# 20k/geodesic_raytracing

Hardware: AMD Instinct MI355X
Metric: Mrays/sec at 3840x2160 Kerr (whole frame: prepass + init + adaptive Verlet + render-data + anisotropic render) (higher is better)
Workload: dtype f32; 1 GPU; kerr_boyer (Boyer-Lindquist rs=1 a=0.45) 3840x2160, camera (0,0,-4,0) fov 90, adaptive_sampling off, prepass on, tol 1e-06, background 4096x2048 RGBA8 10 mips, anisotropy 8; mode=fused, prepass_lookahead=True, prepass_lookahead_depth=1, frames_in_flight=3, prepass=look-ahead on side streams, priming_frames=0, build_key=c6224cf99bf5a7bd-v80s8, counters_tag=kerr_a045_4k, program=substituted (parameters baked in, metric_manager.hpp:153-166), parallelism=single GPU

## Files before the change

### __graft_entry__.py

```python
import os
import subprocess
import sys

ROOT = os.path.dirname(os.path.abspath(__file__))
if ROOT not in sys.path:
    sys.path.insert(0, ROOT)

CONFIG_METRICS = ["minkowski", "schwarzschild", "kerr_boyer", "alcubierre"]
SCRIPT_METRICS = ["minkowski", "schwarzschild", "schwarzschild_adaptive", "kerr_boyer", "double_unequal_kerr", "alcubierre"]


_PRECOMPILE = "import sys; sys.path.insert(0, sys.argv[1]); import geodesic_raytracing_amd as gra; gra.Program.precompile(sys.argv[2])"


def _precompile(job):
    env, argument_string = job
    r = subprocess.run([sys.executable, "-c", _PRECOMPILE, ROOT, argument_string], env=dict(os.environ, **env), capture_output=True, text=True)
    if r.returncode != 0:
        raise RuntimeError(f"precompile of {argument_string[:200]}... failed ({r.returncode}):\n{r.stdout[-2000:]}{r.stderr[-4000:]}")
    return True


def _host_cpus():
    if os.environ.get("MAX_JOBS", "").isdigit() and int(os.environ["MAX_JOBS"]) > 0:
        return int(os.environ["MAX_JOBS"])
    n = len(os.sched_getaffinity(0)) if hasattr(os, "sched_getaffinity") else (os.cpu_count() or 2)
    try:
        with open("/sys/fs/cgroup/cpu.max") as f:
            quota, period = f.read().split()[:2]
        if quota != "max":
            n = min(n, max(1, int(quota) // int(period)))
    except (OSError, ValueError):
        pass
    return n


def build():
    subprocess.check_call(["make", "-C", os.path.join(ROOT, "geodesic_raytracing_amd", "csrc"), "-j8"])
    import geodesic_raytracing_amd as gra
    subprocess.check_call(["make", "-C", os.path.join(ROOT, "examples")])

    cache = os.path.join(ROOT, "geodesic_raytracing_amd", "_cache")
    kernel_dir = os.path.join(ROOT, "geodesic_raytracing_amd", "csrc", "kernels")
    newest_source = max(os.path.getmtime(os.path.join(kernel_dir, f)) for f in os.listdir(kernel_dir))
    if os.path.isdir(cache):
        for f in os.listdir(cache):
            path = os.path.join(cache, f)
            if os.path.getmtime(path) < newest_source:
                os.remove(path)
    jobs = []

    class _Collect:
        @staticmethod
        def precompile(argument_string, **env):
            job = (dict(env), argument_string)
            if job not in jobs:
                jobs.append(job)
    compile_later = _Collect()
    for name in CONFIG_METRICS:
        m = gra.Metric(name)
        compile_later.precompile(m.argument_string())
    compile_later.precompile(gra.Metric("kerr_boyer").argument_string(), GR_TRACE_PAIR_BUILD="1")
    scripts = os.path.join(ROOT, "geodesic_raytracing_amd", "scripts")
    script_metrics = [gra.Metric(name, scripts) for name in SCRIPT_METRICS]
    for m in script_metrics:
        compile_later.precompile(m.argument_string())
        cfg = m.cfg_values(a=0.45) if m.name == "kerr_boyer" else m.cfg_values()
        compile_later.precompile(m.argument_string(features=m.features(adaptive_sampling=0), static=True, cfg_values=cfg))
        if m.name == "kerr_boyer":
            compile_later.precompile(m.argument_string(features=m.features(adaptive_sampling=1, adaptive_sampling_threshold=32.0), static=True, cfg_values=cfg))
        if m.name == "kerr_boyer":
            compile_later.precompile(m.argument_string(features=m.features(adaptive_sampling=0), static=True, cfg_values=m.cfg_values(a=0.9)))
        if m.name == "kerr_boyer":
            for spin in (0.45, 0.9):
                compile_later.precompile(m.argument_string(features=m.features(adaptive_sampling=0), static=True, cfg_values=m.cfg_values(a=spin)) + " -DGR_PARKING")
    import glob as _glob
    for js in sorted(_glob.glob(os.path.join(scripts, "*.js"))):
        m = gra.Metric(os.path.basename(js)[:-3], scripts)
        compile_later.precompile(m.argument_string())
        compile_later.precompile(m.argument_string(features=m.features(adaptive_sampling=1, adaptive_sampling_threshold=32.0), static=True, cfg_values=m.cfg_values()))
    for m in script_metrics:
        if m.name == "alcubierre":
            compile_later.precompile(m.argument_string(features=m.features(adaptive_sampling=0, redshift=1), static=True, cfg_values=m.cfg_values()))

    import glob
    import json
    import numpy as np
    seen = set()
    for f in sorted(glob.glob(os.path.join(ROOT, "tests", "golden", "refscripts", "*.npz"))):
        meta = json.loads(str(np.load(f, allow_pickle=False)["meta"]))
        for text in (meta["argument_string"], meta["argument_string_substituted"]):
            if text not in seen:
                seen.add(text)
                compile_later.precompile(text)
    for f in sorted(glob.glob(os.path.join(ROOT, "tests", "golden", "*.npz")) + glob.glob(os.path.join(ROOT, "tests", "golden", "paths", "*.npz")) + glob.glob(os.path.join(ROOT, "tests", "golden", "paths", "soak", "*.npz"))
                    + glob.glob(os.path.join(ROOT, "tests", "golden", "polar", "*.npz")) + glob.glob(os.path.join(ROOT, "tests", "golden", "soak", "*.npz"))):
        meta = json.loads(str(np.load(f, allow_pickle=False)["meta"]))
        key = (meta["metric"], bool(meta.get("scripts")))
        metric = gra.Metric(meta["metric"], scripts if key[1] else None)
        if key not in seen:
            seen.add(key)
            compile_later.precompile(metric.argument_string())
        if "width" in meta and meta["width"] > 1:
            substituted = metric.argument_string(features=gra.default_features(**meta["features"]), static=True, cfg_values=meta["cfg"])
            if substituted not in seen:
                seen.add(substituted)
                compile_later.precompile(substituted)
                if "near_extreme" in f:
                    compile_later.precompile(substituted + " -cl-fp32-correctly-rounded-divide-sqrt")
                    compile_later.precompile(substituted + " -DGR_REFINED_RECIPROCALS")
    import importlib.util
    spec = importlib.util.spec_from_file_location("fuzz_parity", os.path.join(ROOT, "tests", "fuzz_parity.py"))
    fuzz = importlib.util.module_from_spec(spec)
    spec.loader.exec_module(fuzz)
    fuzz_oracles = []
    for case in fuzz.draw_cases(11, 7):
        metric, cfg, fkw = case[2], case[3], case[7]
        for text in (metric.argument_string(), metric.argument_string(features=gra.default_features(**fkw), static=True, cfg_values=cfg)):
            if text not in seen:
                seen.add(text)
                compile_later.precompile(text)
        fuzz_oracles.append(metric.argument_string())
    spec = importlib.util.spec_from_file_location("uniform_wave_paths", os.path.join(ROOT, "tests", "test_gpu_uniform_wave_paths.py"))
    uniform = importlib.util.module_from_spec(spec)
    spec.loader.exec_module(uniform)
    for name, cfg, features, _position, _ordered, variant in uniform.CASES.values():
        text = uniform.substituted(name, cfg, **features)[3] + (variant[0] if variant else "")
        compile_later.precompile(text)
        compile_later.precompile(text + uniform.WITHOUT)
    tests_dir = os.path.join(ROOT, "tests")
    sys.path.insert(0, tests_dir)
    try:
        spec = importlib.util.spec_from_file_location("render_data_model", os.path.join(tests_dir, "render_data_model.py"))
        render_data_model = importlib.util.module_from_spec(spec)
        spec.loader.exec_module(render_data_model)
    finally:
        sys.path.remove(tests_dir)
    render_data_oracles = [render_data_model.ProgramOf(name).argument_string for name in render_data_model.PROGRAMS]
    for text in render_data_oracles:
        compile_later.precompile(text)
    from concurrent.futures import ThreadPoolExecutor
    workers = max(1, min(len(jobs), _host_cpus() - 1))
    with ThreadPoolExecutor(workers) as pool:
        done = list(pool.map(_precompile, jobs))
    assert all(done) and len(done) == len(jobs)

    from oracle import build_restate, build_ref
    for name in CONFIG_METRICS:
        build_restate.build(gra.Metric(name).argument_string())
    for m in script_metrics:
        build_restate.build(m.argument_string())
    for text in fuzz_oracles + render_data_oracles:
        build_restate.build(text)
    if build_ref.reference_available():
        for name in CONFIG_METRICS:
            build_ref.build_metric(name)
        for m in script_metrics:
            build_ref.build(m.name + "_script", m.argument_string())


def smoke():
    import ctypes
    import numpy as np
    import torch
    import geodesic_raytracing_amd as gra
    from oracle import build_restate
    from oracle.refpipe import OraclePipeline, pack_features

    assert torch.cuda.is_available(), "smoke() needs a GPU: the ray kernels have no CPU fallback"
    W, H = 96, 54
    metric = gra.Metric("kerr_boyer")
    cfg = metric.cfg_values(a=0.45)
    feats = metric.features(adaptive_sampling=0)
    program = gra.Program(metric.argument_string(), 0)
    state = gra.RenderState(W, H, 0)
    bg_np, levels = gra.pack_background(gra.synthetic_background(256, 128))
    device = torch.device("cuda", 0)
    bg = torch.from_numpy(bg_np).to(device)
    out = torch.zeros((H, W, 4), dtype=torch.float32, device=device)
    opts = gra.frame_options(mode=gra.MODE_FUSED, use_prepass=0)
    state.render(program, metric, gra.default_camera(), out.data_ptr(), (bg.data_ptr(), 256, 128, levels), feats, cfg, opts,
                 torch.cuda.current_stream().cuda_stream)
    torch.cuda.synchronize()
    gpu = out.cpu().numpy()

    pipe = OraclePipeline(build_restate.build(metric.argument_string()))
    ref = pipe.frame(W, H, cfg, pack_features(adaptive_sampling=0, max_acceleration_change=metric.info.max_acceleration_change),
                     use_prepass=False, background=(bg_np, levels), nthreads=os.cpu_count() or 1)
    diff = gpu[..., :3] - ref["pixels"][..., :3]
    bad = np.abs(diff).max(axis=2) > 1e-3
    rmse = float(np.sqrt((diff[~bad] ** 2).mean()))
    print(f"smoke: kerr {W}x{H} fused HIP frame vs CPU oracle: rmse {rmse:.2e}, masked {bad.mean() * 100:.2f}% of pixels")
    assert np.isfinite(gpu).all()
    assert bad.mean() <= 0.02, "more than 2% of pixels differ from the oracle by > 1e-3"
    assert rmse < 1e-4, "pixel RMSE vs oracle above 1e-4"


if __name__ == "__main__":
    build()
    print("build ok")
```

### geodesic_raytracing_amd/csrc/kernels/integrator.hip

```cpp

#ifdef ADAPTIVE_PRECISION
#define GR_W_MAX ((float)((W_V1 > W_V2 ? W_V1 : W_V2) > (W_V3 > W_V4 ? W_V3 : W_V4) ? (W_V1 > W_V2 ? W_V1 : W_V2) : (W_V3 > W_V4 ? W_V3 : W_V4)))

__device__ __forceinline__ float acceleration_to_precision(float4 acc, float max_acceleration, float& next_ds) {
    float4 wa = f4(acc.x * (float)(W_V1), acc.y * (float)(W_V2), acc.z * (float)(W_V3), acc.w * (float)(W_V4));
    float current = __builtin_sqrtf(dot4(wa, wa)) * 0.01f;
    current /= GR_W_MAX;
    const float scale = 65536.f;
    float err = max_acceleration;
    float diff = current * scale;
    float floor_diff = err * scale / 1e10f;
    if (diff < floor_diff) diff = floor_diff;
    next_ds = __builtin_sqrtf(err * scale) * __builtin_amdgcn_rsqf(diff);
    return diff;
}
#endif

enum { DS_NONE = 0, DS_SKIP = 1, DS_RETURN = 2 };

#ifdef GR_NO_UNIFORM_WAVE_PATHS
#define GR_UNIFORM_WAVE_PATHS 0
#else
#define GR_UNIFORM_WAVE_PATHS 1
#endif
#if GR_UNIFORM_WAVE_PATHS && defined(GR_RADIUS_EXITS_ORDERED) && !defined(GR_POLAR_R_SQUARED) && !(defined(GR_DISTANCE_SQUARED_OF_GENERIC) && defined(ADAPTIVE_PRECISION))
#define GR_OUTER_BOUNDARY_NEEDS_A_RAY_OUTSIDE 1
#else
#define GR_OUTER_BOUNDARY_NEEDS_A_RAY_OUTSIDE 0
#endif

struct ray_state {
    float4 position, velocity, acceleration;
    float next_ds;
    float running_dlambda_dnew;
    float f_in_x;
    int steps;
    unsigned int tries;
};

enum { RAY_LOST = 0, RAY_TERMINATED = 1 };

__device__ __forceinline__ void integrate_begin(ray_state& s, dfg_t dfg) {
    s.f_in_x = __builtin_fabsf(s.velocity.x);
    s.next_ds = 0.00001f;
#ifdef ADAPTIVE_PRECISION
    (void)acceleration_to_precision(s.acceleration, GET_FEATURE(max_acceleration_change, dfg), s.next_ds);
#endif
    s.running_dlambda_dnew = 1;
    s.steps = 0;
    s.tries = 0;
}

__device__ __forceinline__ float min_f32(float a, float b) { float r; asm("v_min_f32 %0, %1, %2" : "=v"(r) : "v"(a), "v"(b)); return r; }
__device__ __forceinline__ float max_f32(float a, float b) { float r; asm("v_max_f32 %0, %1, %2" : "=v"(r) : "v"(a), "v"(b)); return r; }

__device__ __forceinline__ void overwrite(float4& dst, float4 src) {
    asm volatile("v_mov_b32 %0, %4\n\tv_mov_b32 %1, %5\n\tv_mov_b32 %2, %6\n\tv_mov_b32 %3, %7"
                 : "+v"(dst.x), "+v"(dst.y), "+v"(dst.z), "+v"(dst.w) : "v"(src.x), "v"(src.y), "v"(src.z), "v"(src.w));
}

__device__ __forceinline__ float min_f32_uniform(float uniform, float x) { float r; asm("v_min_f32 %0, %1, %2" : "=v"(r) : "s"(uniform), "v"(x)); return r; }
__device__ __forceinline__ float max_f32_uniform(float uniform, float x) { float r; asm("v_max_f32 %0, %1, %2" : "=v"(r) : "s"(uniform), "v"(x)); return r; }

#ifdef ADAPTIVE_PRECISION
struct step_controller {
    float floor_q, root, singular_q, min_step;
    float root99, floor_step, ambient;
    __device__ __forceinline__ step_controller(float max_acceleration, float min_step_in, float ambient_in) {
        const float scale = 65536.f;
        const float floor_diff = max_acceleration * scale / 1e10f;
        floor_q = floor_diff * floor_diff;
        root = __builtin_sqrtf(max_acceleration * scale);
        root99 = 0.99f * root;
        const float singular = max_acceleration * 10000 * scale;
        singular_q = singular * singular;
        min_step = min_step_in;
        ambient = ambient_in;
        floor_step = __builtin_fminf(min_step_in, ambient_in);
    }
    __device__ __forceinline__ float raw_error_q(float4 acc) const {
        const float k = 0.01f * 65536.f / GR_W_MAX;
        const float wx = acc.x * (float)(W_V1), wy = acc.y * (float)(W_V2), wz = acc.z * (float)(W_V3), ww = acc.w * (float)(W_V4);
        const float d2 = __builtin_fmaf(wx, wx, __builtin_fmaf(wy, wy, __builtin_fmaf(wz, wz, ww * ww)));
        return d2 * (k * k);
    }
    __device__ __forceinline__ float error_q(float4 acc) const { return max_f32_uniform(floor_q, raw_error_q(acc)); }
    __device__ __forceinline__ float suggestion(float q) const { return root * __builtin_amdgcn_rsqf(__builtin_sqrtf(q)); }
    static constexpr bool error_sees_every_component = (float)(W_V1) != 0 && (float)(W_V2) != 0 && (float)(W_V3) != 0 && (float)(W_V4) != 0;
};
#endif

template <bool LIBM> struct trig_flavour { static constexpr bool value = LIBM; };

template <bool RESUMABLE, bool PARKABLE = false>
__device__ __forceinline__ int integrate_pingpong(ray_state& s, cfg_t cfg, dfg_t dfg, unsigned int* attempts, int keep_lanes, bool& paused,
                                                  bool resumed = false, unsigned int park_trips = 0) {
    float4 p0 = s.position, v0 = s.velocity, a0 = s.acceleration;
    float4 p1 = p0, v1 = v0, a1 = a0;
    const bool carried = RESUMABLE || (PARKABLE && resumed);
    if (PARKABLE && !resumed) { s.steps = 0; s.tries = 0; }
    const float f_in_x = carried ? s.f_in_x : __builtin_fabsf(v0.x);
    if (PARKABLE) s.f_in_x = f_in_x;
    const float subambient_precision = 0.5f;
    const float ambient_precision = 0.2f;
    float next_ds = 0.00001f;
#ifdef ADAPTIVE_PRECISION
    const step_controller controller(GET_FEATURE(max_acceleration_change, dfg), GET_FEATURE(min_step, dfg), ambient_precision);
    if (carried) next_ds = s.next_ds;
    else {
        float4 a = a0;
#ifdef IS_CONSTANT_THETA
        a.z = 0;
#endif
        next_ds = controller.suggestion(controller.error_q(a));
    }
    next_ds = min_f32_uniform(ambient_precision, next_ds);
#endif
    const float new_max = GET_FEATURE(max_precision_radius, dfg);
    const float new_min = 3;
    const float universe = GET_FEATURE(universe_size, dfg);
    const bool reparam = GET_FEATURE(reparameterisation, dfg) != 0;
    float running = carried ? s.running_dlambda_dnew : 1.f;
    const int loop_limit = 4096 * 4;
    const unsigned int budget_before = (unsigned int)(loop_limit - (carried ? s.steps : 0));
    unsigned int budget = budget_before;
    unsigned int rejections = 0;
    paused = false;

    auto stop_lost = [&](float4 pos, float4 vel, float4 acc, float run) {
        bool lost = false;
#ifdef HAS_CYLINDRICAL_SINGULARITY
        lost |= pos.y < CYLINDRICAL_TERMINATOR;
#endif
#ifndef UNCONDITIONALLY_NONSINGULAR
        bool runaway = __builtin_fabsf(vel.x / run) > 1000 + f_in_x;
        if (__builtin_expect(__builtin_amdgcn_ballot_w64(runaway) != 0, 0)) {
            asm volatile("; second condition of the runaway test");
            runaway = runaway && __builtin_fabsf(acc.x / run) > 100;
        }
        lost |= runaway;
#endif
        (void)pos; (void)vel; (void)acc; (void)run;
        return lost;
    };
#ifdef GR_POLAR_R_SQUARED
    const float universe2 = universe * universe;
    auto stop_terminated = [&](float4 position, float4 polar) {
        (void)polar;
        const float r2 = gm::polar_radius_squared(position, cfg);
        bool t = r2 >= universe2;
#ifdef SINGULAR
        t |= r2 < (float)(SINGULAR_TERMINATOR) * (float)(SINGULAR_TERMINATOR);
#endif
        return t;
    };
#else
    auto stop_terminated = [&](float4 position, float4 polar) {
        (void)position;
        bool t = __builtin_fabsf(polar.y) >= universe;
#ifdef SINGULAR
        t |= __builtin_fabsf(polar.y) < SINGULAR_TERMINATOR;
#endif
        return t;
    };
#endif
    const float far_offset = ambient_precision - 0.1f * new_max;
#if GR_UNIFORM_WAVE_PATHS
    auto outer_boundary_candidates = [&](float4 pos, float4 polar) {
#ifdef GR_POLAR_R_SQUARED
        (void)polar;
        return __builtin_amdgcn_ballot_w64(gm::polar_radius_squared(pos, cfg) >= universe2);
#else
        (void)pos;
        return __builtin_amdgcn_ballot_w64(__builtin_fabsf(polar.y) >= universe);
#endif
    };
    auto loop_top_candidates = [&](float4 pos, float4 vel, float4 polar, float run) {
        unsigned long long lanes = 0;
#ifdef HAS_CYLINDRICAL_SINGULARITY
        lanes |= __builtin_amdgcn_ballot_w64(pos.y < CYLINDRICAL_TERMINATOR);
#endif
#ifndef UNCONDITIONALLY_NONSINGULAR
        lanes |= __builtin_amdgcn_ballot_w64(__builtin_fabsf(vel.x / run) > 1000 + f_in_x);
#endif
#ifdef SINGULAR
#ifdef GR_POLAR_R_SQUARED
        lanes |= __builtin_amdgcn_ballot_w64(gm::polar_radius_squared(pos, cfg) < (float)(SINGULAR_TERMINATOR) * (float)(SINGULAR_TERMINATOR));
#else
        lanes |= __builtin_amdgcn_ballot_w64(__builtin_fabsf(polar.y) < SINGULAR_TERMINATOR);
#endif
#endif
#if !GR_OUTER_BOUNDARY_NEEDS_A_RAY_OUTSIDE
        lanes |= outer_boundary_candidates(pos, polar);
#endif
        (void)pos; (void)vel; (void)polar; (void)run;
        return lanes;
    };
#endif
    bool pause_wave = false;
    auto attempt = [&](auto libm, float4 position, float4 velocity, float4 acceleration, float4& po, float4& vo, float4& ao, float& ds_used,
                       float& running_before) -> bool {
        if (__builtin_expect(__builtin_usub_overflow(budget, 1u, &budget), 0)) return true;
#ifdef IS_CONSTANT_THETA
        position.z = GR_PIf / 2; velocity.z = 0; acceleration.z = 0;
#endif
        float4 polar = gm::generic_to_spherical(position, cfg);
#ifdef IS_CONSTANT_THETA
        polar.z = GR_PIf / 2;
#endif
#if defined(GR_DISTANCE_SQUARED_OF_GENERIC) && defined(ADAPTIVE_PRECISION)
        const float ar2 = gm::distance_squared_from(position, cfg);
        const bool inside = ar2 < new_max * new_max;
#else
        const float ar = __builtin_fabsf(gm::distance_to_object_from(position, polar, cfg));
        const bool inside = ar < new_max;
#endif
        const unsigned long long inside_lanes = __builtin_amdgcn_ballot_w64(inside);
        const bool wave_inside = inside_lanes != 0;
        (void)wave_inside;
#ifdef ADAPTIVE_PRECISION
        const float near_ds = next_ds;
#else
        const float near_ds = min_f32_uniform(ambient_precision, mixf(ambient_precision, subambient_precision, (clampf(ar, new_min, new_max) - new_min) / (new_max - new_min)));
#endif
#if GR_UNIFORM_WAVE_PATHS
        const bool wave_all_inside = inside_lanes == __builtin_amdgcn_ballot_w64(true);
        unsigned long long leaving = loop_top_candidates(position, velocity, polar, running);
        float ds = near_ds;
        if (!wave_all_inside) {
            asm volatile("; a ray outside the precision radius: the far step, the outer boundary");
#if defined(GR_DISTANCE_SQUARED_OF_GENERIC) && defined(ADAPTIVE_PRECISION)
            const float far_ds = __builtin_fmaf(0.1f, __builtin_sqrtf(ar2), far_offset);
#else
            const float far_ds = __builtin_fmaf(0.1f, ar, far_offset);
#endif
            ds = inside ? near_ds : far_ds;
#if GR_OUTER_BOUNDARY_NEEDS_A_RAY_OUTSIDE
            leaving |= outer_boundary_candidates(position, polar);
#endif
        }
        ds_used = ds;
        running_before = running;
        if (__builtin_expect(leaving != 0, 0)) {
            asm volatile("; a ray at a loop-top exit");
            if (stop_lost(position, velocity, acceleration, running) | stop_terminated(position, polar)) return true;
        }
#else
#if defined(GR_DISTANCE_SQUARED_OF_GENERIC) && defined(ADAPTIVE_PRECISION)
        float far_ds = near_ds;
        if (inside_lanes != __builtin_amdgcn_ballot_w64(true)) {
            asm volatile("; a ray outside the precision radius: the far step");
            far_ds = __builtin_fmaf(0.1f, __builtin_sqrtf(ar2), far_offset);
        }
#else
        const float far_ds = __builtin_fmaf(0.1f, ar, far_offset);
#endif
        const float ds = inside ? near_ds : far_ds;
        ds_used = ds;
        running_before = running;
        if (stop_lost(position, velocity, acceleration, running) | stop_terminated(position, polar)) return true;
#endif
        GR_PROBE_EXTRA_INSTRUCTIONS(ds)
        const float half_ds = 0.5f * ds, half_ds2 = half_ds * ds;
        const float4 next_position = position + velocity * ds + acceleration * half_ds2;
        const float4 predicted = velocity + acceleration * ds;
        float4 next_acceleration = GR_PROBE_ACCELERATION(gm::geodesic_acceleration_with<decltype(libm)::value>(next_position, predicted, cfg), acceleration, predicted, next_position);
        float4 next_velocity = velocity + (acceleration + next_acceleration) * half_ds;
        if (reparam) {
            const float md = __builtin_fmaxf(__builtin_fmaxf(__builtin_fabsf(next_velocity.x), __builtin_fabsf(next_velocity.y)),
                                             __builtin_fmaxf(__builtin_fabsf(next_velocity.z), __builtin_fabsf(next_velocity.w)));
            const float K = 1 / md;
            next_velocity = next_velocity * K;
            next_acceleration = next_acceleration * K * K;
            running *= K;
        }

        po = next_position;
        vo = next_velocity;
        ao = next_acceleration;
        bool dead = false;
#ifdef ADAPTIVE_PRECISION
        float q, nds1;
        unsigned long long rare_lanes;
        if (wave_inside) {
            q = controller.raw_error_q(next_acceleration);
            nds1 = __builtin_amdgcn_fmed3f(controller.root99 * __builtin_amdgcn_rsqf(__builtin_sqrtf(q)), (0.99f * 0.3f) * near_ds, (0.99f * 2.f) * near_ds);
            const float clamped = __builtin_amdgcn_fmed3f(nds1, controller.floor_step, controller.ambient);
            const float threshold = near_ds * (1 / 1.95f);
            rare_lanes = __builtin_amdgcn_ballot_w64(!(__builtin_fmaf(q, 0.f, clamped) >= threshold));
#ifdef SINGULARITY_DETECTION
            rare_lanes |= __builtin_amdgcn_ballot_w64(clamped == controller.floor_step);
#endif
            if (!step_controller::error_sees_every_component) {
                const float poison = (next_velocity.x + next_velocity.y) + (next_velocity.z + next_velocity.w);
                rare_lanes |= __builtin_amdgcn_ballot_w64(!(__builtin_fabsf(poison) <= 3.402823466e+38f));
            }
#if GR_UNIFORM_WAVE_PATHS
            next_ds = clamped;
            if (!wave_all_inside) {
                asm volatile("; a ray outside the precision radius keeps its carried step");
                next_ds = inside ? clamped : near_ds;
            }
#else
            next_ds = inside ? clamped : near_ds;
#endif
        } else {
            const float poison = (next_velocity.x + next_velocity.y) + (next_velocity.z + next_velocity.w);
            q = poison * 0.f;
            nds1 = 0;
            rare_lanes = __builtin_amdgcn_ballot_w64(!(q == q));
        }
        if (__builtin_expect(rare_lanes != 0, 0)) {
            asm volatile("; rejected step, singularity, degenerate state");
            const float nds = max_f32_uniform(controller.min_step, nds1);
#ifdef SINGULARITY_DETECTION
            dead = inside & (q > controller.singular_q) & (nds == controller.min_step);
#endif
            bool reject = inside & (nds < ds * (1 / 1.95f));
            bool degenerate = !(q == q);
            if (!step_controller::error_sees_every_component) {
                const float poison = (next_velocity.x + next_velocity.y) + (next_velocity.z + next_velocity.w);
                degenerate |= !(__builtin_fabsf(poison) <= 3.402823466e+38f);
            }
            dead |= !reject & degenerate;
#ifndef GR_ACCEL_WITHOUT_TRIG
            if (!decltype(libm)::value) {
                dead |= degenerate;
                reject &= !degenerate;
            }
#endif
            if (reject) {
                overwrite(po, position);
                overwrite(vo, velocity);
                overwrite(ao, acceleration);
                asm volatile("v_add_u32 %0, 1, %0\n\tv_add_u32 %1, 1, %1" : "+v"(rejections), "+v"(budget));
            }
        }
#else
        {
            const float poison = (next_velocity.x + next_velocity.y) + (next_velocity.z + next_velocity.w);
            dead = !(__builtin_fabsf(poison) <= 3.402823466e+38f);
        }
#endif
        if (__builtin_expect(dead, 0)) return true;
        if (RESUMABLE) {
            if (__builtin_popcountll(__builtin_amdgcn_ballot_w64(true)) < keep_lanes) { pause_wave = true; return true; }
        }
        return false;
    };

    float exit_ds = 0, exit_running = 1;
    {
        const trig_flavour<false> polynomial;
#if GR_PRIORITY_TRIPS > 0
        unsigned trips = 0, next_level = GR_PRIORITY_TRIPS;
#ifndef GR_PARK_PRIORITY
#define GR_PARK_PRIORITY 0
#endif
        if (PARKABLE && resumed) { __builtin_amdgcn_s_setprio(GR_PARK_PRIORITY); next_level = 0xffffffffu; }
#endif
        unsigned int visit_trips = 0;
        const int park_below = PARKABLE ? __builtin_amdgcn_readfirstlane(keep_lanes) : 0;
        const unsigned int park_after = PARKABLE ? __builtin_amdgcn_readfirstlane(park_trips) : 0u;
        for (;;) {
            float4 p1, v1, a1;
            float ds_used, running_before;
#if GR_PRIORITY_TRIPS > 0
            if (__builtin_expect(++trips == next_level, 0)) {
                if (next_level == GR_PRIORITY_TRIPS) __builtin_amdgcn_s_setprio(1);
                else if (next_level == 2 * GR_PRIORITY_TRIPS) __builtin_amdgcn_s_setprio(2);
                else __builtin_amdgcn_s_setprio(3);
                next_level = next_level < 4 * GR_PRIORITY_TRIPS ? 2 * next_level : 0xffffffffu;
            }
#endif
            if (attempt(polynomial, p0, v0, a0, p1, v1, a1, ds_used, running_before)) {
                if (RESUMABLE && pause_wave) { overwrite(p0, p1); overwrite(v0, v1); overwrite(a0, a1); }
                asm volatile("v_mov_b32 %0, %2\n\tv_mov_b32 %1, %3" : "+v"(exit_ds), "+v"(exit_running) : "v"(ds_used), "v"(running_before));
                break;
            }
            if (attempt(polynomial, p1, v1, a1, p0, v0, a0, ds_used, running_before)) {
                if (!(RESUMABLE && pause_wave)) { overwrite(p0, p1); overwrite(v0, v1); overwrite(a0, a1); }
                asm volatile("v_mov_b32 %0, %2\n\tv_mov_b32 %1, %3" : "+v"(exit_ds), "+v"(exit_running) : "v"(ds_used), "v"(running_before));
                break;
            }
            if (PARKABLE) {
                visit_trips = __builtin_amdgcn_readfirstlane(visit_trips) + 1u;
                if (__builtin_expect(visit_trips >= park_after && __builtin_popcountll(__builtin_amdgcn_ballot_w64(true)) < park_below, 0)) {
                    pause_wave = true;
                    break;
                }
            }
        }
    }
#if GR_PRIORITY_TRIPS > 0
    __builtin_amdgcn_s_setprio(0);
#endif
    float4 position = p0, velocity = v0, acceleration = a0;
#ifdef IS_CONSTANT_THETA
    position.z = GR_PIf / 2; velocity.z = 0; acceleration.z = 0;
#endif
    bool capped, lost_at_top, terminated_at_top;
    auto classify = [&]() {
        capped = budget == 0xffffffffu;
        float4 polar = gm::generic_to_spherical(position, cfg);
#ifdef IS_CONSTANT_THETA
        polar.z = GR_PIf / 2;
#endif
        lost_at_top = stop_lost(position, velocity, acceleration, running);
        terminated_at_top = stop_terminated(position, polar);
    };
    classify();
#if !defined(GR_FAST_TRIG) && !defined(GR_LIBM_TRIG) && !defined(GR_PROBE_NO_SLOW_TRIG)
    if (__builtin_expect(!capped && !pause_wave && !(lost_at_top | terminated_at_top), 0)) {
        const float ds_used = exit_ds;
        float4 polar = gm::generic_to_spherical(position, cfg);
        if (__builtin_fabsf(gm::distance_to_object_from(position, polar, cfg)) < new_max) next_ds = ds_used;
        running = exit_running;
        budget++;
        const trig_flavour<true> precise;
        for (;;) {
            float4 np, nv, na;
            float unused_ds, unused_running;
            const bool leave = attempt(precise, position, velocity, acceleration, np, nv, na, unused_ds, unused_running);
            if (leave && !pause_wave) break;
            position = np; velocity = nv; acceleration = na;
            if (leave) break;
        }
        classify();
    }
#endif
    paused = (RESUMABLE || PARKABLE) && pause_wave;
    const bool left_at_top = !capped && !paused && (lost_at_top | terminated_at_top);
    int result = RAY_LOST;
    if (!paused) {
        const bool finite = degenerate_accumulate(position, degenerate_accumulate(velocity, degenerate_accumulate(acceleration, 0.f))) == 0.f;
        if (!capped && !lost_at_top && terminated_at_top && finite) result = RAY_TERMINATED;
    }
    const unsigned int taken = capped ? budget_before : budget_before - budget - (left_at_top ? 1u : 0u);
    if (RESUMABLE || PARKABLE) { s.next_ds = next_ds; s.steps += (int)taken; s.tries += taken + rejections; }
    s.position = position;
    s.velocity = velocity;
    s.acceleration = acceleration;
    s.running_dlambda_dnew = running;
    if (attempts) *attempts = (RESUMABLE || PARKABLE) ? s.tries : taken + rejections;
    return result;
}

__device__ __forceinline__ int integrate_ray(ray_state& s, cfg_t cfg, dfg_t dfg, unsigned int* attempts) {
    bool paused;
    return integrate_pingpong<false>(s, cfg, dfg, attempts, 0, paused);
}


#ifdef GR_TWO_RAYS_PER_LANE
using gm::pairf;
using gm::pair4;
using gm::splat;
__device__ __forceinline__ pair4 operator+(pair4 a, pair4 b) { return {a.x + b.x, a.y + b.y, a.z + b.z, a.w + b.w}; }
__device__ __forceinline__ pair4 operator*(pair4 a, pairf s) { return {a.x * s, a.y * s, a.z * s, a.w * s}; }
template <int H> __device__ __forceinline__ float4 half_of(pair4 v) {
    return H == 0 ? f4(v.x.x, v.y.x, v.z.x, v.w.x) : f4(v.x.y, v.y.y, v.z.y, v.w.y);
}
__device__ __forceinline__ pair4 pair_of(float4 a, float4 b) {
    pair4 r;
    r.x.x = a.x; r.x.y = b.x; r.y.x = a.y; r.y.y = b.y; r.z.x = a.z; r.z.y = b.z; r.w.x = a.w; r.w.y = b.w;
    return r;
}

#ifdef ADAPTIVE_PRECISION
__device__ __forceinline__ pairf acceleration_to_precision(pair4 acc, float max_acceleration, pairf& next_ds) {
    pair4 wa = {acc.x * (float)(W_V1), acc.y * (float)(W_V2), acc.z * (float)(W_V3), acc.w * (float)(W_V4)};
    pairf d2 = wa.x * wa.x + wa.y * wa.y + wa.z * wa.z + wa.w * wa.w;
    pairf current;
    current.x = __builtin_sqrtf(d2.x); current.y = __builtin_sqrtf(d2.y);
    current = current * 0.01f;
    current = current / GR_W_MAX;
    const float scale = 65536.f;
    float err = max_acceleration;
    pairf diff = current * scale;
    float floor_diff = err * scale / 1e10f;
    if (diff.x < floor_diff) diff.x = floor_diff;
    if (diff.y < floor_diff) diff.y = floor_diff;
    const float root = __builtin_sqrtf(err * scale);
    next_ds.x = root * __builtin_amdgcn_rsqf(diff.x);
    next_ds.y = root * __builtin_amdgcn_rsqf(diff.y);
    return diff;
}
#endif

__device__ __forceinline__ void integrate_pair(pair4& position_io, pair4& velocity_io, pair4 acceleration, pairf& running_out,
                                               bool active0, bool active1, cfg_t cfg, dfg_t dfg, int& result0, int& result1,
                                               unsigned int& tries0, unsigned int& tries1) {
    pair4 position = position_io, velocity = velocity_io;
    pairf f_in_x;
    f_in_x.x = __builtin_fabsf(velocity.x.x); f_in_x.y = __builtin_fabsf(velocity.x.y);
#ifdef IS_CONSTANT_THETA
    position.z = splat(GR_PIf / 2); velocity.z = splat(0.f); acceleration.z = splat(0.f);
#endif
    pairf next_ds = splat(0.00001f);
#ifdef ADAPTIVE_PRECISION
    const float max_accel = GET_FEATURE(max_acceleration_change, dfg);
    const float min_step = GET_FEATURE(min_step, dfg);
    (void)acceleration_to_precision(acceleration, max_accel, next_ds);
#endif
    const float subambient_precision = 0.5f;
    const float ambient_precision = 0.2f;
    const float new_max = GET_FEATURE(max_precision_radius, dfg);
    const float new_min = 3;
    const float universe = GET_FEATURE(universe_size, dfg);
    const bool reparam = GET_FEATURE(reparameterisation, dfg) != 0;
    pairf running = splat(1.f);
    const int loop_limit = 4096 * 4;
    unsigned int t0 = 0, t1 = 0;
    int i0 = 0, i1 = 0;
    bool alive0 = active0, alive1 = active1;

    auto stop_lost = [&](float pos_y, float vel_x_over_run, float acc_x_over_run, float fin, int steps) {
        bool lost = steps >= loop_limit;
#ifdef HAS_CYLINDRICAL_SINGULARITY
        lost |= pos_y < CYLINDRICAL_TERMINATOR;
#endif
#ifndef UNCONDITIONALLY_NONSINGULAR
        lost |= __builtin_fabsf(vel_x_over_run) > 1000 + fin && __builtin_fabsf(acc_x_over_run) > 100;
#endif
        (void)pos_y; (void)vel_x_over_run; (void)acc_x_over_run; (void)fin;
        return lost;
    };
    auto stop_terminated = [&](float polar_y) {
        bool t = __builtin_fabsf(polar_y) >= universe;
#ifdef SINGULAR
        t |= __builtin_fabsf(polar_y) < SINGULAR_TERMINATOR;
#endif
        return t;
    };
    for (;;) {
#ifdef IS_CONSTANT_THETA
        position.z = splat(GR_PIf / 2); velocity.z = splat(0.f); acceleration.z = splat(0.f);
#endif
        pair4 polar = gm::generic_to_spherical(position, cfg);
#ifdef IS_CONSTANT_THETA
        polar.z = splat(GR_PIf / 2);
#endif
        pairf r_value = gm::distance_to_object_from(position, polar, cfg);
        pairf ar;
        ar.x = __builtin_fabsf(r_value.x); ar.y = __builtin_fabsf(r_value.y);
        pairf ds;
#ifdef ADAPTIVE_PRECISION
        ds = next_ds;
#else
        ds.x = mixf(ambient_precision, subambient_precision, (clampf(ar.x, new_min, new_max) - new_min) / (new_max - new_min));
        ds.y = mixf(ambient_precision, subambient_precision, (clampf(ar.y, new_min, new_max) - new_min) / (new_max - new_min));
#endif
        if (ar.x < new_max) ds.x = __builtin_fminf(ds.x, ambient_precision);
        else ds.x = 0.1f * (ar.x - new_max) + ambient_precision;
        if (ar.y < new_max) ds.y = __builtin_fminf(ds.y, ambient_precision);
        else ds.y = 0.1f * (ar.y - new_max) + ambient_precision;

#ifndef UNCONDITIONALLY_NONSINGULAR
        const pairf vq = velocity.x / running, aq = acceleration.x / running;
#else
        const pairf vq = splat(0.f), aq = splat(0.f);
#endif
        alive0 = alive0 && !(stop_lost(position.y.x, vq.x, aq.x, f_in_x.x, i0) | stop_terminated(polar.y.x));
        alive1 = alive1 && !(stop_lost(position.y.y, vq.y, aq.y, f_in_x.y, i1) | stop_terminated(polar.y.y));
        if (!(alive0 | alive1)) break;
        t0 += alive0 ? 1u : 0u;
        t1 += alive1 ? 1u : 0u;

        const pairf half_ds = ds * 0.5f, half_ds2 = half_ds * ds;
        pair4 next_position = position + velocity * ds + acceleration * half_ds2;
        pair4 half_velocity = velocity + acceleration * ds;
        pair4 next_acceleration = GR_PROBE_ACCELERATION_PAIR(gm::geodesic_acceleration(next_position, half_velocity, cfg), acceleration, half_velocity, next_position);
        pair4 next_velocity = velocity + (acceleration + next_acceleration) * half_ds;
        if (reparam) {
            pairf K;
            K.x = 1 / __builtin_fmaxf(__builtin_fmaxf(__builtin_fabsf(next_velocity.x.x), __builtin_fabsf(next_velocity.y.x)),
                                      __builtin_fmaxf(__builtin_fabsf(next_velocity.z.x), __builtin_fabsf(next_velocity.w.x)));
            K.y = 1 / __builtin_fmaxf(__builtin_fmaxf(__builtin_fabsf(next_velocity.x.y), __builtin_fabsf(next_velocity.y.y)),
                                      __builtin_fmaxf(__builtin_fabsf(next_velocity.z.y), __builtin_fabsf(next_velocity.w.y)));
            next_velocity = next_velocity * K;
            next_acceleration = next_acceleration * K * K;
            if (alive0) running.x *= K.x;
            if (alive1) running.y *= K.y;
        }

        bool accept0 = true, accept1 = true;
#ifdef ADAPTIVE_PRECISION
        {
            pairf suggested;
            pairf diff = acceleration_to_precision(next_acceleration, max_accel, suggested);
            const pairf want = suggested * 0.99f, lo = ds * (0.99f * 0.3f), hi = ds * (0.99f * 2.f), back = ds / 1.95f;
            pairf nds;
            nds.x = __builtin_fmaxf(clampf(want.x, lo.x, hi.x), min_step);
            nds.y = __builtin_fmaxf(clampf(want.y, lo.y, hi.y), min_step);
            const bool inside0 = ar.x < new_max, inside1 = ar.y < new_max;
            next_ds.x = inside0 ? nds.x : next_ds.x;
            next_ds.y = inside1 ? nds.y : next_ds.y;
#ifdef SINGULARITY_DETECTION
            const pairf dq = diff / 65536.f;
            alive0 = alive0 & !(inside0 & (nds.x == min_step) & (dq.x > max_accel * 10000));
            alive1 = alive1 & !(inside1 & (nds.y == min_step) & (dq.y > max_accel * 10000));
#endif
            accept0 = !inside0 | !(nds.x < back.x);
            accept1 = !inside1 | !(nds.y < back.y);
            (void)diff;
        }
#endif
        if (alive0 && accept0) {
            position.x.x = next_position.x.x; position.y.x = next_position.y.x; position.z.x = next_position.z.x; position.w.x = next_position.w.x;
            velocity.x.x = next_velocity.x.x; velocity.y.x = next_velocity.y.x; velocity.z.x = next_velocity.z.x; velocity.w.x = next_velocity.w.x;
            acceleration.x.x = next_acceleration.x.x; acceleration.y.x = next_acceleration.y.x; acceleration.z.x = next_acceleration.z.x; acceleration.w.x = next_acceleration.w.x;
            i0++;
            float poison = degenerate_accumulate(half_of<0>(position), degenerate_accumulate(half_of<0>(velocity), 0.f));
            if (reparam) poison = degenerate_accumulate(half_of<0>(acceleration), poison);
            if (!(poison == 0.f)) alive0 = false;
        }
        if (alive1 && accept1) {
            position.x.y = next_position.x.y; position.y.y = next_position.y.y; position.z.y = next_position.z.y; position.w.y = next_position.w.y;
            velocity.x.y = next_velocity.x.y; velocity.y.y = next_velocity.y.y; velocity.z.y = next_velocity.z.y; velocity.w.y = next_velocity.w.y;
            acceleration.x.y = next_acceleration.x.y; acceleration.y.y = next_acceleration.y.y; acceleration.z.y = next_acceleration.z.y; acceleration.w.y = next_acceleration.w.y;
            i1++;
            float poison = degenerate_accumulate(half_of<1>(position), degenerate_accumulate(half_of<1>(velocity), 0.f));
            if (reparam) poison = degenerate_accumulate(half_of<1>(acceleration), poison);
            if (!(poison == 0.f)) alive1 = false;
        }
    }
    {
        pair4 polar = gm::generic_to_spherical(position, cfg);
#ifndef UNCONDITIONALLY_NONSINGULAR
        const pairf vq = velocity.x / running, aq = acceleration.x / running;
#else
        const pairf vq = splat(0.f), aq = splat(0.f);
#endif
        const bool finite0 = degenerate_accumulate(half_of<0>(position), degenerate_accumulate(half_of<0>(velocity), degenerate_accumulate(half_of<0>(acceleration), 0.f))) == 0.f;
        const bool finite1 = degenerate_accumulate(half_of<1>(position), degenerate_accumulate(half_of<1>(velocity), degenerate_accumulate(half_of<1>(acceleration), 0.f))) == 0.f;
        result0 = (!stop_lost(position.y.x, vq.x, aq.x, f_in_x.x, i0) && stop_terminated(polar.y.x) && finite0) ? RAY_TERMINATED : RAY_LOST;
        result1 = (!stop_lost(position.y.y, vq.y, aq.y, f_in_x.y, i1) && stop_terminated(polar.y.y) && finite1) ? RAY_TERMINATED : RAY_LOST;
    }
    position_io = position;
    velocity_io = velocity;
    running_out = running;
    tries0 = t0;
    tries1 = t1;
}
#endif
```

Measured before the change: 1978 Mrays/s.

## Replace per-lane step budget with wave-uniform scalar trip counter in Verlet loop

In the non-resumable integrator, the per-lane budget decrement on every attempt is replaced by a scalar (SGPR) trip counter. The step cap is checked per lane only once the wave passes half the loop limit, and the final budget is rebuilt from the exit trip and the rejection count. The ping-pong step size is also split across two variables so each half of the trip carries its own next_ds, which avoids moving the value between registers. This is meant to cut VALU work and VGPR pressure in the hot loop, at the cost of more complicated step-count accounting near the cap.

```diff
diff --git a/__graft_entry__.py b/__graft_entry__.py
--- a/__graft_entry__.py
+++ b/__graft_entry__.py
@@ -128,6 +128,13 @@
         text = uniform.substituted(name, cfg, **features)[3] + (variant[0] if variant else "")
         compile_later.precompile(text)
         compile_later.precompile(text + uniform.WITHOUT)
+    spec = importlib.util.spec_from_file_location("scalar_budget", os.path.join(ROOT, "tests", "test_gpu_scalar_budget.py"))
+    scalar_budget = importlib.util.module_from_spec(spec)
+    spec.loader.exec_module(scalar_budget)
+    for case in scalar_budget.CASES:
+        text = scalar_budget.program_text(case)[3]
+        compile_later.precompile(text)
+        compile_later.precompile(text, GR_EXTRA_FLAGS=scalar_budget.PER_LANE)
     tests_dir = os.path.join(ROOT, "tests")
     sys.path.insert(0, tests_dir)
     try:
diff --git a/geodesic_raytracing_amd/csrc/kernels/integrator.hip b/geodesic_raytracing_amd/csrc/kernels/integrator.hip
--- a/geodesic_raytracing_amd/csrc/kernels/integrator.hip
+++ b/geodesic_raytracing_amd/csrc/kernels/integrator.hip
@@ -27,6 +27,11 @@
 #define GR_OUTER_BOUNDARY_NEEDS_A_RAY_OUTSIDE 1
 #else
 #define GR_OUTER_BOUNDARY_NEEDS_A_RAY_OUTSIDE 0
+#endif
+#ifdef GR_PER_LANE_BUDGET
+#define GR_WAVE_UNIFORM_BUDGET 0
+#else
+#define GR_WAVE_UNIFORM_BUDGET 1
 #endif
 
 struct ray_state {
@@ -91,6 +96,7 @@
 #endif
 
 template <bool LIBM> struct trig_flavour { static constexpr bool value = LIBM; };
+template <unsigned int WHICH> struct attempt_of_trip { static constexpr unsigned int value = WHICH; };
 
 template <bool RESUMABLE, bool PARKABLE = false>
 __device__ __forceinline__ int integrate_pingpong(ray_state& s, cfg_t cfg, dfg_t dfg, unsigned int* attempts, int keep_lanes, bool& paused,
@@ -125,6 +131,10 @@
     const unsigned int budget_before = (unsigned int)(loop_limit - (carried ? s.steps : 0));
     unsigned int budget = budget_before;
     unsigned int rejections = 0;
+    constexpr bool uniform_budget = GR_WAVE_UNIFORM_BUDGET && !RESUMABLE && !PARKABLE;
+    static_assert(loop_limit % 2 == 0, "the scalar step-cap test reads the trip count");
+    unsigned int trips = 0;
+    unsigned long long cap_candidates = 0;
     paused = false;
 
     auto stop_lost = [&](float4 pos, float4 vel, float4 acc, float run) {
@@ -198,9 +208,19 @@
     };
 #endif
     bool pause_wave = false;
-    auto attempt = [&](auto libm, float4 position, float4 velocity, float4 acceleration, float4& po, float4& vo, float4& ao, float& ds_used,
-                       float& running_before) -> bool {
-        if (__builtin_expect(__builtin_usub_overflow(budget, 1u, &budget), 0)) return true;
+    auto attempt = [&](auto libm, auto which_of_trip, float4 position, float4 velocity, float4 acceleration, float4& po, float4& vo, float4& ao,
+                       float step_in, float& step_out, float& ds_used, float& running_before) -> bool {
+        constexpr bool scalar_cap = uniform_budget && !decltype(libm)::value;
+        const bool past_limit = scalar_cap && trips > (unsigned int)(loop_limit / 2);
+        auto stop_capped = [&]() { return 2u * trips - 1u + decltype(which_of_trip)::value - rejections > (unsigned int)loop_limit; };
+        constexpr bool cap_with_the_exits = scalar_cap && GR_UNIFORM_WAVE_PATHS;
+        (void)past_limit; (void)stop_capped; (void)cap_with_the_exits;
+        if (scalar_cap) {
+            if (!cap_with_the_exits && __builtin_expect(past_limit, 0)) {
+                asm volatile("; past the wave's 16 384th attempt: the step cap, lane by lane");
+                if (stop_capped()) return true;
+            }
+        } else if (__builtin_expect(__builtin_usub_overflow(budget, 1u, &budget), 0)) return true;
 #ifdef IS_CONSTANT_THETA
         position.z = GR_PIf / 2; velocity.z = 0; acceleration.z = 0;
 #endif
@@ -219,7 +239,7 @@
         const bool wave_inside = inside_lanes != 0;
         (void)wave_inside;
 #ifdef ADAPTIVE_PRECISION
-        const float near_ds = next_ds;
+        const float near_ds = step_in;
 #else
         const float near_ds = min_f32_uniform(ambient_precision, mixf(ambient_precision, subambient_precision, (clampf(ar, new_min, new_max) - new_min) / (new_max - new_min)));
 #endif
@@ -241,8 +261,10 @@
         }
         ds_used = ds;
         running_before = running;
+        if (cap_with_the_exits) leaving |= cap_candidates;
         if (__builtin_expect(leaving != 0, 0)) {
             asm volatile("; a ray at a loop-top exit");
+            if (cap_with_the_exits && cap_candidates != 0 && stop_capped()) return true;
             if (stop_lost(position, velocity, acceleration, running) | stop_terminated(position, polar)) return true;
         }
 #else
@@ -296,19 +318,20 @@
                 rare_lanes |= __builtin_amdgcn_ballot_w64(!(__builtin_fabsf(poison) <= 3.402823466e+38f));
             }
 #if GR_UNIFORM_WAVE_PATHS
-            next_ds = clamped;
+            step_out = clamped;
             if (!wave_all_inside) {
                 asm volatile("; a ray outside the precision radius keeps its carried step");
-                next_ds = inside ? clamped : near_ds;
-            }
-#else
-            next_ds = inside ? clamped : near_ds;
+                step_out = inside ? clamped : near_ds;
+            }
+#else
+            step_out = inside ? clamped : near_ds;
 #endif
         } else {
             const float poison = (next_velocity.x + next_velocity.y) + (next_velocity.z + next_velocity.w);
             q = poison * 0.f;
             nds1 = 0;
             rare_lanes = __builtin_amdgcn_ballot_w64(!(q == q));
+            step_out = near_ds;
         }
         if (__builtin_expect(rare_lanes != 0, 0)) {
             asm volatile("; rejected step, singularity, degenerate state");
@@ -333,7 +356,8 @@
                 overwrite(po, position);
                 overwrite(vo, velocity);
                 overwrite(ao, acceleration);
-                asm volatile("v_add_u32 %0, 1, %0\n\tv_add_u32 %1, 1, %1" : "+v"(rejections), "+v"(budget));
+                if (scalar_cap) asm volatile("v_add_u32 %0, 1, %0" : "+v"(rejections));
+                else asm volatile("v_add_u32 %0, 1, %0\n\tv_add_u32 %1, 1, %1" : "+v"(rejections), "+v"(budget));
             }
         }
 #else
@@ -350,10 +374,21 @@
     };
 
     float exit_ds = 0, exit_running = 1;
+    unsigned int exit_entered = 0;
     {
         const trig_flavour<false> polynomial;
+        const attempt_of_trip<0> first;
+        const attempt_of_trip<1> second;
+#if GR_WAVE_UNIFORM_BUDGET && defined(ADAPTIVE_PRECISION)
+        float step1 = next_ds;
+#define GR_STEP_OF_SET_1 step1
+#define GR_LEAVE_STEP_IN_SET_0 asm volatile("v_mov_b32 %0, %1" : "+v"(next_ds) : "v"(step1));
+#else
+#define GR_STEP_OF_SET_1 next_ds
+#define GR_LEAVE_STEP_IN_SET_0
+#endif
 #if GR_PRIORITY_TRIPS > 0
-        unsigned trips = 0, next_level = GR_PRIORITY_TRIPS;
+        unsigned next_level = GR_PRIORITY_TRIPS;
 #ifndef GR_PARK_PRIORITY
 #define GR_PARK_PRIORITY 0
 #endif
@@ -372,15 +407,22 @@
                 else __builtin_amdgcn_s_setprio(3);
                 next_level = next_level < 4 * GR_PRIORITY_TRIPS ? 2 * next_level : 0xffffffffu;
             }
-#endif
-            if (attempt(polynomial, p0, v0, a0, p1, v1, a1, ds_used, running_before)) {
+#else
+            if (uniform_budget) ++trips;
+#endif
+            if (uniform_budget && GR_UNIFORM_WAVE_PATHS && __builtin_expect(trips > (unsigned int)(loop_limit / 2), 0))
+                asm volatile("s_mov_b64 %0, -1" : "+s"(cap_candidates));
+            if (attempt(polynomial, first, p0, v0, a0, p1, v1, a1, next_ds, GR_STEP_OF_SET_1, ds_used, running_before)) {
                 if (RESUMABLE && pause_wave) { overwrite(p0, p1); overwrite(v0, v1); overwrite(a0, a1); }
+                GR_LEAVE_STEP_IN_SET_0
                 asm volatile("v_mov_b32 %0, %2\n\tv_mov_b32 %1, %3" : "+v"(exit_ds), "+v"(exit_running) : "v"(ds_used), "v"(running_before));
+                if (uniform_budget) asm volatile("v_mov_b32 %0, %1" : "+v"(exit_entered) : "s"(2u * trips - 1u));
                 break;
             }
-            if (attempt(polynomial, p1, v1, a1, p0, v0, a0, ds_used, running_before)) {
+            if (attempt(polynomial, second, p1, v1, a1, p0, v0, a0, GR_STEP_OF_SET_1, next_ds, ds_used, running_before)) {
                 if (!(RESUMABLE && pause_wave)) { overwrite(p0, p1); overwrite(v0, v1); overwrite(a0, a1); }
                 asm volatile("v_mov_b32 %0, %2\n\tv_mov_b32 %1, %3" : "+v"(exit_ds), "+v"(exit_running) : "v"(ds_used), "v"(running_before));
+                if (uniform_budget) asm volatile("v_mov_b32 %0, %1" : "+v"(exit_entered) : "s"(2u * trips));
                 break;
             }
             if (PARKABLE) {
@@ -392,9 +434,12 @@
             }
         }
     }
+#undef GR_STEP_OF_SET_1
+#undef GR_LEAVE_STEP_IN_SET_0
 #if GR_PRIORITY_TRIPS > 0
     __builtin_amdgcn_s_setprio(0);
 #endif
+    if (uniform_budget) budget = budget_before - exit_entered + rejections;
     float4 position = p0, velocity = v0, acceleration = a0;
 #ifdef IS_CONSTANT_THETA
     position.z = GR_PIf / 2; velocity.z = 0; acceleration.z = 0;
@@ -421,7 +466,7 @@
         for (;;) {
             float4 np, nv, na;
             float unused_ds, unused_running;
-            const bool leave = attempt(precise, position, velocity, acceleration, np, nv, na, unused_ds, unused_running);
+            const bool leave = attempt(precise, attempt_of_trip<0>(), position, velocity, acceleration, np, nv, na, next_ds, next_ds, unused_ds, unused_running);
             if (leave && !pause_wave) break;
             position = np; velocity = nv; acceleration = na;
             if (leave) break;
```

Measured after the change: 1997 Mrays/s, median of 6. About the same (+1.0%).
